# PacificBiosciences/pb-StarPhase

Measured on AMD Instinct MI355X. Metric: HiFi reads/sec diplotyped (HLA+CYP2D6), higher is better.
Workload: dtype int32; 1 GPU; BASELINE configs[1] + configs[2] as ONE sample per step: HLA-A/-B 10000 HiFi reads vs IMGT/HLA v0.14.1 (11,199 DNA alleles) + CYP2D6 2000 targeted reads (39 templates), the six configs[2] scenarios in turn; a new sample uploaded every step; reads -> diplotypes; hla_reads=10000, cyp2d6_reads=2000, cyp2d6_lanes=6, hla_lanes=2, cyp2d6_consensus=launch pairs

## Files before the change

### pb-starphase_amd/csrc/sp_consensus.hip

```cpp
#include "sp_internal.h"
#include <atomic>
#include <cstdlib>
#include "sp_wfa.hip.h"
#include <algorithm>
#include <cstddef>
#include <cstring>
#include <map>
#include <string>

namespace {

constexpr int CB = 64;
constexpr int CH = 32;
#ifndef SP_K8_WAVES
#define SP_K8_WAVES 8
#endif
#ifndef SP_K8_MIN_WAVES
#define SP_K8_MIN_WAVES 4
#endif
constexpr int CWAVES = SP_K8_WAVES;
#ifndef SP_K8_DBG_READS
#define SP_K8_DBG_READS 16384
#endif
#define SP_K8_DBG_LAUNCHES (4194304 / SP_K8_DBG_READS)
// ... 581 lines not shown
    }
    return pi;
}
template <int MAXP> __device__ __forceinline__ int block_problem(const ConsBatchT<MAXP>& B) { return block_problem<MAXP>(B, (int)blockIdx.x); }

__device__ __forceinline__ size_t state_plane(int node, int slot, int cons) { return (size_t)((node * 2 + slot) * 2 + cons); }

__device__ __forceinline__ int read_cost(const Dwfa& a0, const Dwfa& a1, bool dualrun) {
    int c = -1;
    if (a0.flags & F_ACTIVE) c = a0.e;
    if (dualrun && (a1.flags & F_ACTIVE) && (c < 0 || a1.e < c)) c = a1.e;
    return c < 0 ? 0 : c;
}

template <int MAXP>
__device__ __forceinline__ void cons_step_body(const ConsBatchT<MAXP>& B, const int wrow) {
    __shared__ unsigned long long lv[2][CW + 1];
    __shared__ uint32_t le[2][CW + 1];
    __shared__ unsigned long long ll[2][CW];
    __shared__ uint32_t lc[CW + 1], lr[CW + 1];
    __shared__ uint8_t cwin[2][CWIN + CW];
    __shared__ uint32_t rwin[CWAVES][2][RWORDS + 2];
    __shared__ uint32_t cpk[2][(CWIN + CW) / 16 + 2];
    __shared__ ActScratch act[CWAVES];
    __shared__ CWork wk_s;
    const int pi = block_problem<MAXP>(B);
    const ConsParams P = B.p[pi];
    const bool coh = B.sync != nullptr;
    if (coh) {
        for (int x = threadIdx.x; x < (int)(sizeof(CWork) / 4); x += blockDim.x) ((uint32_t*)&wk_s)[x] = coh_load(((const uint32_t*)P.work) + x);
        __syncthreads();
    }
    const CWork* Wp = coh ? &wk_s : P.work + wrow;
    const int mode = Wp->mode;
    if (P.work->done || mode == M_NONE) return;
    if (wrow > 0 && P.n_blocks > DIRECT_BLOCKS) return;
    if (B.step_t && threadIdx.x == 0) atomicMin(&B.step_t[2 * pi], (unsigned long long)wall_clock64());
    const int lane = threadIdx.x & 63, wave = threadIdx.x >> 6;
    const int T = Wp->T, n = (mode == M_WINDOW || mode == M_EXPAND) ? Wp->n : 0;
    const int pre = mode == M_EXPAND ? n : 0;
    const int node = Wp->node, in_slot = Wp->in_slot;
    const int dual_in = Wp->dual, split_at = Wp->split_at;
    const int go0 = Wp->go[0], go1 = Wp->go[1];
    const int n_kids = (mode == M_EXPAND || mode == M_WINDOW) ? Wp->n_kids : 0;
    const uint8_t* Cn = P.C + (size_t)node * 2 * P.cs;
    for (int x = threadIdx.x; x < 2 * (CW + 1); x += blockDim.x) { (&lv[0][0])[x] = 0; (&le[0][0])[x] = 0; }
    for (int x = threadIdx.x; x < 2 * CW; x += blockDim.x) (&ll[0][0])[x] = 0;
    for (int x = threadIdx.x; x < CW + 1; x += blockDim.x) { lc[x] = 0; lr[x] = 0; }
    const int w0 = T - CWIN;
    for (int x = threadIdx.x; x < 2 * (CWIN + CW); x += blockDim.x) {
        const int i = x / (CWIN + CW), y = x % (CWIN + CW), pos = w0 + y;
        uint8_t v = 0;
        if (pos >= T) v = (pos - T < n) ? Wp->spec[dual_in ? i : 0][pos - T] : 0;
        else if (pos >= 0) v = coh_load((i == 1 && dual_in && pos >= split_at) ? &Cn[(size_t)P.cs + pos] : &Cn[pos]);
        cwin[i][y] = v;
    }
    __syncthreads();
    constexpr int CPW = (CWIN + CW) / 16 + 2;
    for (int x = threadIdx.x; x < 2 * CPW; x += blockDim.x) {
        const int i = x / CPW, w = x % CPW;
        uint32_t word = 0;
        for (int b = 0; b < 16; ++b) { const int y = w * 16 + b; if (y < CWIN + n) word |= (uint32_t)(cwin[i][y] & 3u) << (b << 1); }
        cpk[i][w] = word;
    }
    __syncthreads();
    const size_t plane = (size_t)B.total;
    for (int rr = 0; rr < P.rpw; ++rr) {
        const int r = (((int)blockIdx.x - P.first_block) * CWAVES + wave) * P.rpw + rr;
        if (r >= P.n) break;
        const size_t g = (size_t)P.first + r;
#ifdef SP_K8_TIMING
        const long long wt0 = wall_clock64();
        if (lane == 0) { act[wave].tk[0] = act[wave].tk[1] = act[wave].tk[2] = act[wave].tk[3] = 0; }
#endif
        const ReadInfo ri = B.info[g];
        ReadView rv; rv.w = ri.w; rv.np = ri.np; rv.n = ri.n;
        if (lane == 0) act[wave].staged = nullptr;
        Dwfa d0, d1;
        d0.H = SP_NEG; d0.e = 0; d0.c0 = 0; d0.flags = 0; d1 = d0;
        if (mode == M_INIT) {
            if (ri.off < 0) { d0.flags = F_ACTIVE | ((P.et && rv.n == 0) ? F_FINISHED : 0); d0.H = lane == CH ? 0 : SP_NEG; }
        } else {
            const size_t p0 = state_plane(node, in_slot, 0) * plane + g;
            const ConsMeta m0 = B.meta[p0];
            d0.H = h_load(B.H, p0 * CB + lane); d0.e = m0.e; d0.c0 = m0.c0; d0.flags = m0.flags;
            if (dual_in) {
                const size_t p1 = state_plane(node, in_slot, 1) * plane + g;
                const ConsMeta m1 = B.meta[p1];
                d1.H = h_load(B.H, p1 * CB + lane); d1.e = m1.e; d1.c0 = m1.c0; d1.flags = m1.flags;
            }
        }
        int rbase = 0;
        {
            int lo = 0x7FFFFFFF;
            if (d0.flags & F_ACTIVE) { const int x = T - d0.c0 - CB; lo = x < lo ? x : lo; }
            if (dual_in && (d1.flags & F_ACTIVE)) { const int x = T - d1.c0 - CB; lo = x < lo ? x : lo; }
            if (lo == 0x7FFFFFFF || lo < 0) lo = 0;
            rbase = (lo >> 4) << 4;
            const int w_first = rbase >> 4, w_last = (rv.n + 15) >> 4;
            if (lane < RWORDS + 2) {
                const int w = w_first + lane;
                rwin[wave][0][lane] = w <= w_last + 1 ? rv.w[w] : 0u;
                rwin[wave][1][lane] = (rv.np && w <= w_last + 1) ? rv.np[w] : 0u;
            }
            spw::wave_lds_sync();
        }
        auto rb = [&](int h) -> int {
            const int x = h - rbase;
            if ((unsigned)x < (unsigned)(RWORDS * 16)) {
                const uint32_t sh = (uint32_t)(x & 15) << 1;
                if ((rwin[wave][1][x >> 4] >> sh) & 1u) return 4;
                return (int)((rwin[wave][0][x >> 4] >> sh) & 3u);
            }
            return read_base(rv, h);
        };
        auto vote = [&](const Dwfa& a, const Dwfa& o, bool dualrun, int i, int col, int slot) {
            if (!(a.flags & F_ACTIVE) || (a.flags & (F_FINISHED | F_LOST))) return;
            if (dualrun && (o.flags & F_ACTIVE) && !(o.flags & F_LOST) && o.e < a.e) return;
            const int Tl = col - a.c0, k = lane - CH;
            const bool tip = a.H >= 0 && a.H + k == Tl;
            const int code = (tip && a.H < rv.n) ? rb(a.H) : 5;
            int dc = 0; unsigned long long word = 0;
#pragma unroll
            for (int b = 0; b < 4; ++b) { const bool s = __ballot(code == b) != 0; dc += s; word |= s ? (1ull << (16 * b)) : 0ull; }
            const bool ended = __ballot(tip) != 0 && __ballot(code == 4) == 0;
            if (lane == 0) {
                if (dc) atomicAdd(&lv[i][slot], word * vote_units(dc));
                else if (ended) atomicAdd(&le[i][slot], 12u);
            }
        };
        bool use_pk = mode == M_WINDOW;
        auto extender = [&](const ConsAccess& cacc, int i) {
            return [&cacc, i, &rb, wave, rbase, w0, lane, &use_pk, &rv](Dwfa& d, int Tc) {
                const int k = lane - CH;
                for (;;) {
                    int left = rv.n - d.H; { const int l2 = Tc - (d.H + k); left = l2 < left ? l2 : left; }
                    const bool go = d.H >= 0 && left > 0;
                    int nm = 0; bool more = false;
                    if (go) {
                        const int xr = d.H - rbase, yc = d.c0 + d.H + k - w0;
                        if (use_pk && xr >= 0 && xr < RWORDS * 16 && yc >= 0 && yc < CWIN + CW) {
                            const uint32_t a = __builtin_amdgcn_alignbit(rwin[wave][0][(xr >> 4) + 1], rwin[wave][0][xr >> 4], (uint32_t)(xr & 15) << 1);
                            const uint32_t nn = __builtin_amdgcn_alignbit(rwin[wave][1][(xr >> 4) + 1], rwin[wave][1][xr >> 4], (uint32_t)(xr & 15) << 1);
                            const uint32_t b = __builtin_amdgcn_alignbit(cpk[i][(yc >> 4) + 1], cpk[i][yc >> 4], (uint32_t)(yc & 15) << 1);
                            const uint32_t xo = a ^ b, mm = ((xo | (xo >> 1)) | nn) & 0x55555555u;
                            nm = mm ? (__builtin_ctz(mm) >> 1) : 16;
                            nm = nm < left ? nm : left;
                            more = nm == 16 && left > 16;
                        } else {
                            const int x = rb(d.H);
                            nm = (x < 4 && x == cacc.at(d.c0 + d.H + k)) ? 1 : 0;
                            more = nm == 1 && left > 1;
                        }
                        d.H += nm;
                    }
                    if (!__ballot(more)) break;
                }
            };
        };
        auto column = [&](Dwfa& a0, Dwfa& a1, bool dualrun, int g0, int g1, int nb0, int nb1, int len, const ConsAccess& c0a, const ConsAccess& c1a) {
            if (g0) {
                if (a0.flags & F_ACTIVE) { if (!(a0.flags & (F_FINISHED | F_LOST))) dwfa_push_t(a0, rv.n, rb, extender(c0a, c0a.i), len - a0.c0, nb0, P.et, lane); }
                else if (ri.off == len) { a0 = activate_late(rv, c0a, &act[wave], B.memo + 2 * ((size_t)wrow * plane + g), ri.off0, len, P.window, P.cmp_len, P.et, lane); spw::wave_lds_sync(); }
            }
            if (dualrun && g1) {
                if (a1.flags & F_ACTIVE) { if (!(a1.flags & (F_FINISHED | F_LOST))) dwfa_push_t(a1, rv.n, rb, extender(c1a, c1a.i), len - a1.c0, nb1, P.et, lane); }
                else if (ri.off == len) { a1 = activate_late(rv, c1a, &act[wave], B.memo + 2 * ((size_t)wrow * plane + g), ri.off0, len, P.window, P.cmp_len, P.et, lane); spw::wave_lds_sync(); }
            }
            if (dualrun) {
                const int both = (a0.flags & F_ACTIVE) && (a1.flags & F_ACTIVE) && !(a0.flags & F_LOST) && !(a1.flags & F_LOST);
                if (both) {
                    if (a0.e > a1.e + P.delta) a0.flags |= F_LOST;
                    else if (a1.e > a0.e + P.delta) a1.flags |= F_LOST;
// ... 1130 lines not shown
        }
    }
#ifdef SP_K8_SEARCH_TICKS
    if (tid == 0) { ss.ticks[0] += 100 * ts_iters - (tk1 - tk0); ss.ticks[1] += ts_pick - (tk2 - tk1); ss.ticks[3] += ts_block - (wall_clock64() - tk3); }
#endif
    __syncthreads();
    for (int x = tid; x < NQ * NODE_HEAD_WORDS; x += blockDim.x)
        put(&((uint32_t*)&P.nodes[x / NODE_HEAD_WORDS])[x % NODE_HEAD_WORDS], ((const uint32_t*)&nh[x / NODE_HEAD_WORDS])[x % NODE_HEAD_WORDS], coh);
    for (int x = tid; x < NQ * NODE_TAPE_WORDS; x += blockDim.x) {
        const int k = x / NODE_TAPE_WORDS, w = x % NODE_TAPE_WORDS;
        if (tape_word_used(nh[k], w)) ((uint32_t*)&P.nodes[k])[NODE_HEAD_WORDS + w] = ((const uint32_t*)&nh[k])[NODE_HEAD_WORDS + w];
    }
    for (int x = tid; x < n_orders * (int)(sizeof(CWork) / 4); x += blockDim.x) put(&((uint32_t*)P.work)[x], ((const uint32_t*)wks)[x], coh);
    for (int x = tid; x < (int)(sizeof(CSearch) / 4); x += blockDim.x) ((uint32_t*)P.srch)[x] = ((const uint32_t*)&ss)[x];
    for (int x = tid; x < proc_words; x += blockDim.x) ((uint32_t*)P.processed)[x] = ((const uint32_t*)proc)[x];
    if (tid == 0 && B.prog) {
        __hip_atomic_store(B.prog + 2 * pi, (uint32_t)wk.pad, __ATOMIC_RELAXED, __HIP_MEMORY_SCOPE_SYSTEM);
        if (wk.done) __hip_atomic_store(B.prog + 2 * pi + 1, 1u, __ATOMIC_RELAXED, __HIP_MEMORY_SCOPE_SYSTEM);
    }
}

template <int MAXP>
__global__ void __launch_bounds__(1024) cons_control_kernel(ConsBatchT<MAXP> B) { cons_control_body<MAXP>(B); }

constexpr long long PERSIST_TIMEOUT = 400000000ll;
constexpr double PERSIST_READY_S = 0.5;
__device__ __forceinline__ bool persist_wait(const uint32_t* word, uint32_t at_least, uint32_t* abort_word) {
    const long long t0 = wall_clock64();
    for (uint32_t spins = 1;; ++spins) {
        if (__hip_atomic_load(word, __ATOMIC_RELAXED, __HIP_MEMORY_SCOPE_AGENT) >= at_least) return true;
        __builtin_amdgcn_s_sleep(1);
        if ((spins & 63u) == 0) {
            if (__hip_atomic_load(abort_word, __ATOMIC_RELAXED, __HIP_MEMORY_SCOPE_AGENT)) return false;
            if (wall_clock64() - t0 > PERSIST_TIMEOUT) { __hip_atomic_store(abort_word, 1u, __ATOMIC_RELAXED, __HIP_MEMORY_SCOPE_AGENT); return false; }
        }
    }
}

template <int MAXP>
__global__ void __launch_bounds__(CWAVES * SP_WAVE, SP_K8_MIN_WAVES) cons_step_persist_kernel(ConsBatchT<MAXP> B) {
    __shared__ int go_on;
    const int pi = block_problem<MAXP>(B);
    uint32_t* sy = B.sync + 4 * pi; uint32_t* abort_word = B.sync + 4 * B.n_prob;
    for (uint32_t k = 1;; ++k) {
        if (threadIdx.x == 0) go_on = persist_wait(sy + 0, k - 1, abort_word) ? 1 : 0;
        __syncthreads();
        if (!go_on) break;
        if (coh_load(&B.p[pi].work->done)) break;
        cons_step_body<MAXP>(B, 0);
        asm volatile("s_waitcnt vmcnt(0)" ::: "memory");
        __syncthreads();
        if (threadIdx.x == 0) __hip_atomic_fetch_add(sy + 1, 1u, __ATOMIC_RELAXED, __HIP_MEMORY_SCOPE_AGENT);
    }
}

template <int MAXP>
__global__ void __launch_bounds__(1024) cons_control_persist_kernel(ConsBatchT<MAXP> B) {
    __shared__ int go_on;
    const int pi = blockIdx.x;
    const uint32_t nb = (uint32_t)B.p[pi].n_blocks;
    uint32_t* sy = B.sync + 4 * pi; uint32_t* abort_word = B.sync + 4 * B.n_prob;
    if (threadIdx.x == 0 && B.ready) __hip_atomic_fetch_add(B.ready, 1u, __ATOMIC_RELAXED, __HIP_MEMORY_SCOPE_SYSTEM);
    for (uint32_t k = 1;; ++k) {
        if (threadIdx.x == 0) {
            go_on = persist_wait(sy + 1, nb * k, abort_word) ? 1 : 0;
            if (go_on && k > B.step_cap) { __hip_atomic_store(abort_word, 2u, __ATOMIC_RELAXED, __HIP_MEMORY_SCOPE_AGENT); go_on = 0; }
        }
        __syncthreads();
        if (!go_on) break;
        __builtin_amdgcn_fence(__ATOMIC_ACQUIRE, "agent");
        cons_control_body<MAXP>(B);
        asm volatile("s_waitcnt vmcnt(0)" ::: "memory");
        __syncthreads();
        const bool done = coh_load(&B.p[pi].work->done) != 0;
        if (threadIdx.x == 0) __hip_atomic_store(sy + 0, k, __ATOMIC_RELAXED, __HIP_MEMORY_SCOPE_AGENT);
        if (done) break;
    }
    if (threadIdx.x == 0 && B.prog) {
        const uint32_t ab = __hip_atomic_load(abort_word, __ATOMIC_RELAXED, __HIP_MEMORY_SCOPE_AGENT);
        if (ab) __hip_atomic_store(B.prog + 2 * pi + 1, 1u + ab, __ATOMIC_RELAXED, __HIP_MEMORY_SCOPE_SYSTEM);
    }
}

__global__ void cons_setup_kernel(ConsSetup S, ReadInfo* __restrict__ info) {
    const int r = blockIdx.x * blockDim.x + threadIdx.x;
    if (r >= S.n) return;
    const uint32_t rid = S.idx ? S.idx[r] : (uint32_t)r;
    ReadInfo ri;
    ri.w = S.reads.words + S.reads.word_off[rid];
    ri.np = S.reads.nplane ? S.reads.nplane + S.reads.word_off[rid] : nullptr;
    ri.n = S.reads.len[rid]; ri.off0 = S.offsets ? S.offsets[r] : -1; ri.off = ri.off0 < 0 ? -1 : ri.off0 + max(0, min(S.cmp_len, ri.n)); ri.pad = 0;
    info[S.first + r] = ri;
}

__global__ void cons_setup_many_kernel(const ConsSetup* __restrict__ S, int n_prob, int total, ReadInfo* __restrict__ info) {
    const int t = blockIdx.x * blockDim.x + threadIdx.x;
    if (t >= total) return;
    int lo = 0, hi = n_prob - 1;
    while (lo < hi) { const int mid = (lo + hi + 1) >> 1; if (S[mid].first <= t) lo = mid; else hi = mid - 1; }
    while (lo + 1 < n_prob && S[lo].n == 0 && S[lo + 1].first <= t) ++lo;
    const ConsSetup& q = S[lo];
    const int r = t - q.first;
    if (r < 0 || r >= q.n) return;
    const uint32_t rid = q.idx ? q.idx[r] : (uint32_t)r;
    ReadInfo ri;
    ri.w = q.reads.words + q.reads.word_off[rid];
    ri.np = q.reads.nplane ? q.reads.nplane + q.reads.word_off[rid] : nullptr;
    ri.n = q.reads.len[rid]; ri.off0 = q.offsets ? q.offsets[r] : -1; ri.off = ri.off0 < 0 ? -1 : ri.off0 + max(0, min(q.cmp_len, ri.n)); ri.pad = 0;
    info[t] = ri;
}

template <int MAXP>
__global__ void __launch_bounds__(SP_WAVE) cons_finalize_kernel(ConsBatchT<MAXP> B, uint8_t* is_cons1, int32_t* score1, int32_t* score2) {
    const int vblock = (int)blockIdx.x / CWAVES, wave = (int)blockIdx.x % CWAVES;
    const int pi = block_problem<MAXP>(B, vblock);
    const ConsParams P = B.p[pi];
    const int lane = threadIdx.x;
    const int best = P.srch->best_node;
    const size_t plane = (size_t)B.total;
    if (vblock == P.first_block && wave == 0) {
        for (int x = threadIdx.x; x < (int)(sizeof(CSearch) / 4); x += blockDim.x) ((uint32_t*)P.out_srch)[x] = ((const uint32_t*)P.srch)[x];
        if (threadIdx.x == 0) {
            ConsRes r; r.best = best; r.dual = 0; r.split_at = -1; r.len1 = r.len2 = 0; r.pad = 0;
            if (best >= 0) { const CNode* x = P.nodes + best; r.dual = x->dual; r.split_at = x->split_at; r.len1 = x->len[0]; r.len2 = x->dual ? x->len[1] : 0; }
            *P.out_res = r;
        }
        if (best >= 0) {
            const uint8_t* src = P.C + (size_t)best * 2 * P.cs;
#pragma unroll
            for (int i = 0; i < 2; ++i) {
                const uint32_t* s4 = reinterpret_cast<const uint32_t*>(src + (size_t)i * P.cs);
                uint8_t* dst = P.out_cons + (size_t)i * P.cap;
                for (int x = (int)threadIdx.x * 4; x < P.cap; x += (int)blockDim.x * 4) {
                    const uint32_t w = s4[x >> 2];
#pragma unroll
                    for (int q = 0; q < 4; ++q) if (x + q < P.cap) dst[x + q] = (uint8_t)(w >> (8 * q));
                }
            }
        }
    }
    for (int rr = 0; rr < P.rpw; ++rr) {
        const int r = ((vblock - P.first_block) * CWAVES + wave) * P.rpw + rr;
        if (r >= P.n) break;
        const size_t g = (size_t)P.first + r;
        int sc[2] = { -1, -1 };
        if (best >= 0) {
            const CNode* x = P.nodes + best;
            const int n = B.info[g].n, cur = x->cur, dual = x->dual;
#pragma unroll
            for (int i = 0; i < 2; ++i) {
                if (i == 1 && !dual) continue;
                const size_t p = state_plane(best, cur, i) * plane + g;
                const ConsMeta m = B.meta[p];
                if (!(m.flags & F_ACTIVE) || (m.flags & F_LOST)) continue;
                int e = m.e;
                if (!P.et) {
                    const int h = h_load(B.H, p * CB + lane), k = lane - CH;
                    int rest = (h >= 0 && h + k == x->len[i] - m.c0) ? n - h : (1 << 30);
#pragma unroll
                    for (int o = 32; o > 0; o >>= 1) { const int other = __shfl_xor(rest, o); rest = other < rest ? other : rest; }
                    if (rest < (1 << 30)) e += rest;
                }
                sc[i] = e;
            }
        }
        if (lane == 0) {
            score1[g] = sc[0]; score2[g] = sc[1];
            is_cons1[g] = !(sc[1] >= 0 && (sc[0] < 0 || sc[1] < sc[0]));
        }
    }
}

}

constexpr int PERSIST_MAX_BATCHES = 4;
struct PersistLease {
    int device = -1, taken = 0;
    static std::atomic<int>& used(int device) { static std::atomic<int> u[64]; return u[device & 63]; }
// ... 120 lines not shown
    const size_t zero_nodes = place(zero_bytes, sizeof(CNode) * NQ * n_prob), zero_proc = place(zero_bytes, proc_bytes), zero_info = place(zero_bytes, sizeof(ReadInfo) * total), zero_memo = place(zero_bytes, sizeof(PlaceMemo) * 2 * total * (size_t)(1 + nside));
    const size_t zero_sync = place(zero_bytes, sizeof(uint32_t) * (4 * (size_t)n_prob + 4));
    uint8_t* d_in = (uint8_t*)sp_pool(ctx, "cons_in", in_bytes + 16); uint8_t* h_in = (uint8_t*)sp_host_pool(ctx, "cons_in", in_bytes + 16);
    uint8_t* d_out = (uint8_t*)sp_pool(ctx, "cons_out", out_bytes + 16); uint8_t* h_out = (uint8_t*)sp_host_pool(ctx, "cons_out", out_bytes + 16);
    uint8_t* d_zero = (uint8_t*)sp_pool(ctx, "cons_zero", zero_bytes + 16);
    if (!d_in || !h_in || !d_out || !h_out || !d_zero) return sp_fail(ctx, SP_ERR_OUT_OF_MEMORY, "sp_consensus staging");
    uint32_t* d_idx = (uint32_t*)(d_in + in_idx); int32_t* d_off = (int32_t*)(d_in + in_off);
    uint8_t* d_C = (uint8_t*)sp_pool(ctx, "cons_C", c_bytes);
    CWork* d_work = (CWork*)(d_in + in_work);
    CSearch* d_srch = (CSearch*)(d_in + in_srch);
    CNode* d_nodes = (CNode*)(d_zero + zero_nodes);
    uint32_t* d_la = (uint32_t*)sp_pool(ctx, "cons_la", sizeof(uint32_t) * (size_t)NQ * 2 * CW * 4 * n_prob);
    uint8_t* d_proc = d_zero + zero_proc;
    ReadInfo* d_info = (ReadInfo*)(d_zero + zero_info);
    B.memo = (PlaceMemo*)(d_zero + zero_memo);
    B.sync = persist_rpw ? (uint32_t*)(d_zero + zero_sync) : nullptr;
    B.info = d_info; B.total = (int)total;
    B.H = (uint16_t*)sp_pool(ctx, "cons_H", sizeof(uint16_t) * planes * total * CB);
    B.meta = (ConsMeta*)sp_pool(ctx, "cons_meta", sizeof(ConsMeta) * planes * total);
    const size_t wblocks = (size_t)n_blocks + (size_t)NWORK * n_prob;
    B.PV = (unsigned long long*)sp_pool(ctx, "cons_pv", sizeof(unsigned long long) * wblocks * 2 * (CW + 1));
    B.PE = (uint32_t*)sp_pool(ctx, "cons_pe", sizeof(uint32_t) * wblocks * 2 * (CW + 1));
    B.PL = (unsigned long long*)sp_pool(ctx, "cons_pl", sizeof(unsigned long long) * wblocks * 2 * CW);
    B.PC = (uint32_t*)sp_pool(ctx, "cons_pc", sizeof(uint32_t) * wblocks * (CW + 1));
    B.PR = (uint32_t*)sp_pool(ctx, "cons_pr", sizeof(uint32_t) * wblocks * (CW + 1));
    B.Q = (uint32_t*)sp_pool(ctx, "cons_q", sizeof(uint32_t) * (size_t)n_clusters * QE);
#ifdef SP_K8_TIMING
    B.dbg = (unsigned long long*)sp_pool(ctx, "cons_dbg", (size_t)SP_K8_DBG_LAUNCHES * SP_K8_DBG_READS * 8);
    (void)hipMemsetAsync(B.dbg, 0, (size_t)SP_K8_DBG_LAUNCHES * SP_K8_DBG_READS * 8, st);
#endif
    uint8_t* d_is1 = d_out + out_is1;
    int32_t* d_sc = (int32_t*)(d_out + out_sc);
    B.step_t = nullptr;
    if (ctx->profiling) {
        B.step_t = (unsigned long long*)sp_pool(ctx, "cons_step_t", sizeof(unsigned long long) * 2 * n_prob);
        if (B.step_t) {
            std::vector<unsigned long long> init((size_t)2 * n_prob);
            for (uint32_t p = 0; p < n_prob; ++p) { init[2 * p] = ~0ull; init[2 * p + 1] = 0ull; }
            unsigned long long* h_st = (unsigned long long*)sp_host_pool(ctx, "cons_step_t", sizeof(unsigned long long) * 2 * n_prob);
            if (h_st) { std::memcpy(h_st, init.data(), init.size() * 8); (void)hipMemcpyAsync(B.step_t, h_st, init.size() * 8, hipMemcpyHostToDevice, st); } else B.step_t = nullptr;
        }
    }
    uint32_t* h_prog = (uint32_t*)sp_host_pool(ctx, "cons_prog", sizeof(uint32_t) * 2 * n_prob);
    if (!h_prog) return sp_fail(ctx, SP_ERR_OUT_OF_MEMORY, "sp_consensus progress words");
    std::memset(h_prog, 0, sizeof(uint32_t) * 2 * n_prob);
    { void* dp = nullptr; SP_HIP_CHECK(ctx, hipHostGetDevicePointer(&dp, h_prog, 0)); B.prog = (uint32_t*)dp; }
    CWork* h_work = (CWork*)sp_host_pool(ctx, "cons_work", sizeof(CWork) * n_prob);
    CWork* h_work0 = (CWork*)(h_in + in_work); CSearch* h_srch0 = (CSearch*)(h_in + in_srch);
    const CSearch* h_srch = (const CSearch*)(h_out + out_srch);
    if (!d_idx || !d_off || !d_C || !d_work || !d_srch || !d_nodes || !d_la || !d_proc || !d_info || !B.H || !B.meta || !B.PV || !B.PE || !B.PL || !B.PC || !B.PR || !B.Q ||
        !h_work)
        return sp_fail(ctx, SP_ERR_OUT_OF_MEMORY, "sp_consensus buffers");
    for (uint32_t p = 0; p < n_prob; ++p) {
        setup[p].idx = probs[p].read_idx ? d_idx + idx_at[p] : nullptr;
        setup[p].offsets = probs[p].offsets ? d_off + off_at[p] : nullptr; setup[p].cmp_len = probs[p].cfg.offset_compare_length; setup[p].pad_ = 0;
        hp[p].C = d_C + c_at[p]; hp[p].work = d_work + (size_t)p * NWORK; hp[p].srch = d_srch + p; hp[p].nodes = d_nodes + (size_t)p * NQ;
        hp[p].la = d_la + (size_t)p * NQ * 2 * CW * 4; hp[p].processed = d_proc + proc_at[p];
        hp[p].acc_block = n_blocks + (int)p * NWORK;
        hp[p].out_cons = d_out + out_cons[p]; hp[p].out_res = (ConsRes*)(d_out + out_res) + p; hp[p].out_srch = (CSearch*)(d_out + out_srch) + p;
    }
    if constexpr (MAXP == 0) {
        std::memcpy(h_in + in_probs, hp.data(), sizeof(ConsParams) * n_prob);
        std::memcpy(h_in + in_bp, block_prob.data(), sizeof(int) * block_prob.size());
        std::memcpy(h_in + in_cp, cluster_prob.data(), sizeof(int) * cluster_prob.size());
        B.p = (const ConsParams*)(d_in + in_probs); B.block_prob = (const int*)(d_in + in_bp); B.cluster_prob = (const int*)(d_in + in_cp);
    } else {
        for (uint32_t p = 0; p < n_prob; ++p) B.p[p] = hp[p];
    }
    for (uint32_t p = 0; p < n_prob; ++p) {
        std::memset(&h_work0[(size_t)p * NWORK], 0, sizeof(CWork) * NWORK);
        CWork& w = h_work0[(size_t)p * NWORK]; w.mode = M_INIT; w.node = 0; w.in_slot = 0; w.split_at = -1;
        CSearch& s = h_srch0[p]; std::memset(&s, 0, sizeof s); s.best_node = -1; s.inflight = -1;
        const sp_cons_config& cf = probs[p].cfg;
        s.max_queue = cf.max_queue_size > 0 ? std::min(cf.max_queue_size, NQ - MAXKIDS - 2) : 20;
        s.per_size = cf.max_capacity_per_size > 0 ? std::min(cf.max_capacity_per_size, 255) : 10;
        s.wo_constraint = cf.max_nodes_wo_constraint > 0 ? cf.max_nodes_wo_constraint : 1000;
    }
    if (!h_idx.empty()) std::memcpy(h_in + in_idx, h_idx.data(), sizeof(uint32_t) * h_idx.size());
    if (!h_off.empty()) std::memcpy(h_in + in_off, h_off.data(), sizeof(int32_t) * h_off.size());
    if (n_prob > 8) std::memcpy(h_in + in_setup, setup.data(), sizeof(ConsSetup) * n_prob);
    SP_HIP_CHECK(ctx, hipMemcpyAsync(d_in, h_in, in_bytes, hipMemcpyHostToDevice, st));
    SP_HIP_CHECK(ctx, hipMemsetAsync(d_zero, 0, zero_bytes, st));
    {
        const size_t nb = (size_t)n_blocks, np = (size_t)n_prob * NWORK;
        SP_HIP_CHECK(ctx, hipMemsetAsync(B.PV + nb * 2 * (CW + 1), 0, sizeof(unsigned long long) * np * 2 * (CW + 1), st));
        SP_HIP_CHECK(ctx, hipMemsetAsync(B.PE + nb * 2 * (CW + 1), 0, sizeof(uint32_t) * np * 2 * (CW + 1), st));
        SP_HIP_CHECK(ctx, hipMemsetAsync(B.PL + nb * 2 * CW, 0, sizeof(unsigned long long) * np * 2 * CW, st));
        SP_HIP_CHECK(ctx, hipMemsetAsync(B.PC + nb * (CW + 1), 0, sizeof(uint32_t) * np * (CW + 1), st));
        SP_HIP_CHECK(ctx, hipMemsetAsync(B.PR + nb * (CW + 1), 0, sizeof(uint32_t) * np * (CW + 1), st));
    }
    if (n_prob > 8) hipLaunchKernelGGL(cons_setup_many_kernel, dim3((unsigned)((total + 255) / 256)), dim3(256), 0, st, (const ConsSetup*)(d_in + in_setup), (int)n_prob, (int)total, d_info);
    else for (uint32_t p = 0; p < n_prob; ++p)
        if (setup[p].n) hipLaunchKernelGGL(cons_setup_kernel, dim3((setup[p].n + 255) / 256), dim3(256), 0, st, setup[p], d_info);

    B.nside = persist_rpw ? 0 : nside;
    B.k8_compound = ctx->k8_compound;
    const dim3 grid((uint32_t)n_blocks, (uint32_t)(1 + B.nside)), block(CWAVES * SP_WAVE);
    const bool one_round = n_blocks <= (ctx->num_cus + ctx->num_cus / 4) * (8 / CWAVES);
    size_t proc_lds = ((size_t)max_cap + 2 + 15) & ~(size_t)15;
    {
        hipFuncAttributes fa;
        SP_HIP_CHECK(ctx, hipFuncGetAttributes(&fa, (const void*)cons_control_kernel<MAXP>));
        if (fa.sharedSizeBytes + proc_lds > 160 * 1024) return sp_fail(ctx, SP_ERR_TOO_LONG, "sp_consensus: cap must stay below ~65,000");
    }
    SP_HIP_CHECK(ctx, hipFuncSetAttribute((const void*)cons_control_kernel<MAXP>, hipFuncAttributeMaxDynamicSharedMemorySize, (int)proc_lds));
    uint64_t pairs = 0;
    bool persist_ran = false;
    hm.mark("host:k8_prologue");
    double t_launch = 0.0;
    {
        ProfScope ps(ctx, "cons_steps", total);
        const uint64_t limit = (uint64_t)64 * (uint64_t)(max_cap + 2) + 1024;
        const uint32_t ahead = 3;
        bool need_reduce = false;
        for (uint32_t p = 0; p < n_prob; ++p) need_reduce = need_reduce || hp[p].n_blocks > DIRECT_BLOCKS;
        volatile uint32_t* prog = h_prog;
        bool finished = false;
        if (persist_rpw) {
            if (!ctx->ctl_stream && hipStreamCreateWithFlags(&ctx->ctl_stream, hipStreamNonBlocking) != hipSuccess) return sp_fail(ctx, SP_ERR_HIP, "sp_consensus: control stream");
            if (!ctx->ev_fork && (hipEventCreateWithFlags(&ctx->ev_fork, hipEventDisableTiming) != hipSuccess || hipEventCreateWithFlags(&ctx->ev_join, hipEventDisableTiming) != hipSuccess))
                return sp_fail(ctx, SP_ERR_HIP, "sp_consensus: events");
            SP_HIP_CHECK(ctx, hipFuncSetAttribute((const void*)cons_control_persist_kernel<MAXP>, hipFuncAttributeMaxDynamicSharedMemorySize, (int)proc_lds));
            SP_HIP_CHECK(ctx, hipEventRecord(ctx->ev_fork, st));
            SP_HIP_CHECK(ctx, hipStreamWaitEvent(ctx->ctl_stream, ctx->ev_fork, 0));
            uint32_t* h_ready = (uint32_t*)sp_host_pool(ctx, "cons_ready", 64);
            if (!h_ready) return sp_fail(ctx, SP_ERR_OUT_OF_MEMORY, "sp_consensus ready word");
            *(volatile uint32_t*)h_ready = 0;
            { void* dp = nullptr; SP_HIP_CHECK(ctx, hipHostGetDevicePointer(&dp, h_ready, 0)); B.ready = (uint32_t*)dp; }
            B.step_cap = (uint32_t)std::min<uint64_t>(limit, 0xFFFFFFFFull);
            auto drain = [&]() { (void)hipStreamSynchronize(ctx->ctl_stream); (void)hipStreamSynchronize(st); };
            hipLaunchKernelGGL(cons_control_persist_kernel<MAXP>, dim3(n_prob), dim3(1024), proc_lds, ctx->ctl_stream, B);
            bool all_ready = true;
            {
                const auto t_wait = std::chrono::steady_clock::now();
                const bool forced = std::getenv("SP_K8_FORCE_READY_TIMEOUT") != nullptr;
                while (forced || *(volatile uint32_t*)h_ready < n_prob) {
                    __builtin_ia32_pause();
                    if (forced || std::chrono::duration<double>(std::chrono::steady_clock::now() - t_wait).count() > PERSIST_READY_S) { all_ready = false; break; }
                }
            }
            if (all_ready) {
                hipLaunchKernelGGL(cons_step_persist_kernel<MAXP>, dim3((uint32_t)n_blocks), block, 0, st, B);
                const hipError_t e1 = hipGetLastError();
                const hipError_t e2 = e1 == hipSuccess ? hipEventRecord(ctx->ev_join, ctx->ctl_stream) : e1;
                const hipError_t e3 = e2 == hipSuccess ? hipStreamWaitEvent(st, ctx->ev_join, 0) : e2;
                if (e3 != hipSuccess) {
                    const uint32_t one = 1;
                    if (!ctx->copy_stream) (void)hipStreamCreateWithFlags(&ctx->copy_stream, hipStreamNonBlocking);
                    if (ctx->copy_stream) { (void)hipMemcpyAsync(B.sync + 4 * n_prob, &one, 4, hipMemcpyHostToDevice, ctx->copy_stream); (void)hipStreamSynchronize(ctx->copy_stream); }
                    drain();
                    return sp_fail(ctx, SP_ERR_HIP, std::string("sp_consensus: persistent launch: ") + hipGetErrorString(e3));
                }
                finished = true; persist_ran = true;
            } else {
                const uint32_t one = 1;
                if (!ctx->copy_stream && hipStreamCreateWithFlags(&ctx->copy_stream, hipStreamNonBlocking) != hipSuccess) { drain(); return sp_fail(ctx, SP_ERR_HIP, "sp_consensus: copy stream"); }
                (void)hipMemcpyAsync(B.sync + 4 * n_prob, &one, 4, hipMemcpyHostToDevice, ctx->copy_stream);
                (void)hipStreamSynchronize(ctx->copy_stream);
                (void)hipStreamSynchronize(ctx->ctl_stream);
                lease.give_back();
                ctx->k8_persist_failures += 1; ctx->k8_persist_backoff = 64;
                ctx->warning = "persistent consensus kernels: the control workgroups of a batch found no free CUs within " + std::to_string(PERSIST_READY_S) +
                               " s (another process on this device?): the batch ran launch by launch, and so will the next 64";
                (void)hipMemsetAsync(B.sync, 0, sizeof(uint32_t) * (4 * (size_t)n_prob + 1), st);
                std::memset(h_prog, 0, sizeof(uint32_t) * 2 * n_prob);
                B.sync = nullptr; B.ready = nullptr;
                persist_rpw = 0;
            }
        }
        while (!finished) {
            const auto tl0 = std::chrono::steady_clock::now();
            if (one_round) hipLaunchKernelGGL(cons_step_wide_kernel<MAXP>, grid, block, 0, st, B);
            else hipLaunchKernelGGL(cons_step_kernel<MAXP>, grid, block, 0, st, B);
            if (need_reduce) hipLaunchKernelGGL(cons_reduce_kernel<MAXP>, dim3((uint32_t)n_clusters * RSLICES), dim3(512), 0, st, B);
            hipLaunchKernelGGL(cons_control_kernel<MAXP>, dim3(n_prob), dim3(1024), proc_lds, st, B);
            t_launch += std::chrono::duration<double, std::milli>(std::chrono::steady_clock::now() - tl0).count();
// ... 336 lines not shown
```

Measured before the change: 361,800 reads/s.

## Skip dead read states early and fuse accumulator clears into setup kernels

In the consensus step kernel, a wave now checks whether both DWFA states of a read are finished, lost or out of window before loading the 64-lane H vectors. If none need work, it only forwards the metadata to the window slot and to each child node, then skips the read. Separately, five hipMemsetAsync calls that zeroed the per-problem accumulators are replaced by a grid-stride clear inside the setup kernels, which removes several launches per batch. The early exit has to reproduce the state propagation exactly, so it carries some correctness risk. The per-problem clears for small batches also rely on hp[p].acc_block, which must be laid out consistently with the old contiguous region.

```diff
diff --git a/pb-starphase_amd/csrc/sp_consensus.hip b/pb-starphase_amd/csrc/sp_consensus.hip
--- a/pb-starphase_amd/csrc/sp_consensus.hip
+++ b/pb-starphase_amd/csrc/sp_consensus.hip
@@ -687,13 +687,37 @@
             if (ri.off < 0) { d0.flags = F_ACTIVE | ((P.et && rv.n == 0) ? F_FINISHED : 0); d0.H = lane == CH ? 0 : SP_NEG; }
         } else {
             const size_t p0 = state_plane(node, in_slot, 0) * plane + g;
+            const size_t p1 = state_plane(node, in_slot, 1) * plane + g;
             const ConsMeta m0 = B.meta[p0];
-            d0.H = h_load(B.H, p0 * CB + lane); d0.e = m0.e; d0.c0 = m0.c0; d0.flags = m0.flags;
-            if (dual_in) {
-                const size_t p1 = state_plane(node, in_slot, 1) * plane + g;
-                const ConsMeta m1 = B.meta[p1];
-                d1.H = h_load(B.H, p1 * CB + lane); d1.e = m1.e; d1.c0 = m1.c0; d1.flags = m1.flags;
-            }
+            d0.e = m0.e; d0.c0 = m0.c0; d0.flags = m0.flags;
+            if (dual_in) { const ConsMeta m1 = B.meta[p1]; d1.e = m1.e; d1.c0 = m1.c0; d1.flags = m1.flags; }
+            {
+                const int t_hi = T + n + 1;
+                const bool dead0 = (d0.flags & F_ACTIVE) ? (d0.flags & (F_FINISHED | F_LOST)) != 0 : !(ri.off > T && ri.off <= t_hi);
+                const bool dead1 = !dual_in || ((d1.flags & F_ACTIVE) ? (d1.flags & (F_FINISHED | F_LOST)) != 0 : !(ri.off > T && ri.off <= t_hi));
+                const bool both = dual_in && (d0.flags & F_ACTIVE) && (d1.flags & F_ACTIVE) && !((d0.flags | d1.flags) & F_LOST);
+                const bool pending = both && (d0.e > d1.e + P.delta || d1.e > d0.e + P.delta);
+                if (__builtin_amdgcn_readfirstlane((int)(dead0 && dead1 && !pending))) {
+                    auto put_meta = [&](const Dwfa& a, int nd, int slot, int i) { ConsMeta m; m.e = a.e; m.c0 = a.c0; m.flags = a.flags; m.pad = 0; B.meta[state_plane(nd, slot, i) * plane + g] = m; };
+                    if (lane == 0) {
+                        if (mode == M_WINDOW) { put_meta(d0, node, in_slot ^ 1, 0); if (dual_in) put_meta(d1, node, in_slot ^ 1, 1); }
+                        for (int k = 0; k < n_kids; ++k) {
+                            const int kn = Wp->kid_node[k], ksplit = Wp->kid_split[k];
+                            put_meta(d0, kn, 0, 0);
+                            if (dual_in || ksplit) put_meta(ksplit ? d0 : d1, kn, 0, 1);
+                        }
+                    }
+#if defined(SP_K8_TIMING) && !defined(SP_K8_DBG_PARTS)
+                    if (B.dbg && lane == 0 && Wp->pad < SP_K8_DBG_LAUNCHES && g < SP_K8_DBG_READS) {
+                        const unsigned long long dt = (unsigned long long)(wall_clock64() - wt0);
+                        B.dbg[(size_t)Wp->pad * SP_K8_DBG_READS + g] = (dt > 0xFFFFFF ? 0xFFFFFFull : dt) | ((unsigned long long)mode << 24) | ((unsigned long long)(n > 511 ? 511 : n) << 45);
+                    }
+#endif
+                    continue;
+                }
+            }
+            d0.H = h_load(B.H, p0 * CB + lane);
+            if (dual_in) d1.H = h_load(B.H, p1 * CB + lane);
         }
         int rbase = 0;
         {
@@ -1990,7 +2014,17 @@
     }
 }
 
-__global__ void cons_setup_kernel(ConsSetup S, ReadInfo* __restrict__ info) {
+struct AccClear { unsigned long long* pv; uint32_t* pe; unsigned long long* pl; uint32_t* pc; uint32_t* pr; int blocks; };
+__device__ __forceinline__ void acc_clear(const AccClear& A) {
+    const size_t t = (size_t)blockIdx.x * blockDim.x + threadIdx.x, nt = (size_t)gridDim.x * blockDim.x;
+    const size_t nv = (size_t)A.blocks * 2 * (CW + 1), nl = (size_t)A.blocks * 2 * CW, nc = (size_t)A.blocks * (CW + 1);
+    for (size_t i = t; i < nv; i += nt) { A.pv[i] = 0ull; A.pe[i] = 0u; }
+    for (size_t i = t; i < nl; i += nt) A.pl[i] = 0ull;
+    for (size_t i = t; i < nc; i += nt) { A.pc[i] = 0u; A.pr[i] = 0u; }
+}
+
+__global__ void cons_setup_kernel(ConsSetup S, ReadInfo* __restrict__ info, AccClear A) {
+    acc_clear(A);
     const int r = blockIdx.x * blockDim.x + threadIdx.x;
     if (r >= S.n) return;
     const uint32_t rid = S.idx ? S.idx[r] : (uint32_t)r;
@@ -2001,7 +2035,8 @@
     info[S.first + r] = ri;
 }
 
-__global__ void cons_setup_many_kernel(const ConsSetup* __restrict__ S, int n_prob, int total, ReadInfo* __restrict__ info) {
+__global__ void cons_setup_many_kernel(const ConsSetup* __restrict__ S, int n_prob, int total, ReadInfo* __restrict__ info, AccClear A) {
+    acc_clear(A);
     const int t = blockIdx.x * blockDim.x + threadIdx.x;
     if (t >= total) return;
     int lo = 0, hi = n_prob - 1;
@@ -2288,16 +2323,15 @@
     SP_HIP_CHECK(ctx, hipMemcpyAsync(d_in, h_in, in_bytes, hipMemcpyHostToDevice, st));
     SP_HIP_CHECK(ctx, hipMemsetAsync(d_zero, 0, zero_bytes, st));
     {
-        const size_t nb = (size_t)n_blocks, np = (size_t)n_prob * NWORK;
-        SP_HIP_CHECK(ctx, hipMemsetAsync(B.PV + nb * 2 * (CW + 1), 0, sizeof(unsigned long long) * np * 2 * (CW + 1), st));
-        SP_HIP_CHECK(ctx, hipMemsetAsync(B.PE + nb * 2 * (CW + 1), 0, sizeof(uint32_t) * np * 2 * (CW + 1), st));
-        SP_HIP_CHECK(ctx, hipMemsetAsync(B.PL + nb * 2 * CW, 0, sizeof(unsigned long long) * np * 2 * CW, st));
-        SP_HIP_CHECK(ctx, hipMemsetAsync(B.PC + nb * (CW + 1), 0, sizeof(uint32_t) * np * (CW + 1), st));
-        SP_HIP_CHECK(ctx, hipMemsetAsync(B.PR + nb * (CW + 1), 0, sizeof(uint32_t) * np * (CW + 1), st));
-    }
-    if (n_prob > 8) hipLaunchKernelGGL(cons_setup_many_kernel, dim3((unsigned)((total + 255) / 256)), dim3(256), 0, st, (const ConsSetup*)(d_in + in_setup), (int)n_prob, (int)total, d_info);
-    else for (uint32_t p = 0; p < n_prob; ++p)
-        if (setup[p].n) hipLaunchKernelGGL(cons_setup_kernel, dim3((setup[p].n + 255) / 256), dim3(256), 0, st, setup[p], d_info);
+        auto acc_at = [&](size_t blk, int blocks) { AccClear a; a.pv = B.PV + blk * 2 * (CW + 1); a.pe = B.PE + blk * 2 * (CW + 1); a.pl = B.PL + blk * 2 * CW; a.pc = B.PC + blk * (CW + 1); a.pr = B.PR + blk * (CW + 1); a.blocks = blocks; return a; };
+        if (n_prob > 8) {
+            const size_t words = (size_t)n_prob * NWORK * 2 * (CW + 1);
+            const size_t threads = std::max<size_t>(total, std::min<size_t>((words + 15) / 16, (size_t)4096 * 256));
+            hipLaunchKernelGGL(cons_setup_many_kernel, dim3((unsigned)((threads + 255) / 256)), dim3(256), 0, st, (const ConsSetup*)(d_in + in_setup), (int)n_prob, (int)total, d_info,
+                               acc_at((size_t)n_blocks, (int)n_prob * NWORK));
+        } else for (uint32_t p = 0; p < n_prob; ++p)
+            hipLaunchKernelGGL(cons_setup_kernel, dim3(std::max(1, (setup[p].n + 255) / 256)), dim3(256), 0, st, setup[p], d_info, acc_at((size_t)hp[p].acc_block, NWORK));
+    }
 
     B.nside = persist_rpw ? 0 : nside;
     B.k8_compound = ctx->k8_compound;
```

After: 330,100 reads/s. -8.8%, worse.
